# OminiX-ai/OminiX-MLX

Measured on AMD Instinct MI355X. Metric: decode_tokens_per_sec, higher is better.
Workload: dtype bf16

## Files before the change

### ominix-mlx_amd/csrc/attn_step.hip

```cpp
#include <algorithm>

#include "attn.hpp"
#include "act16.hpp"
#include "gemv_parts.hpp"
#include "granule.hpp"
#include "launch_timing.hpp"

namespace omx {

namespace {

constexpr int kBlock = 512;
constexpr int kWaves = 8;

template <int N>
__device__ __forceinline__ float swap_halves(float v) {
    if (N == 16) return dpp_f<0x128>(v);
    return dpp_f<0x1B>(dpp_f<kDppHalfMirror>(v));
}

template <bool F16 = false>
__device__ __forceinline__ void unpack8(const u32x4 r, float (&x)[8]) {
#pragma unroll
    for (int e = 0; e < 4; ++e) {
        x[2 * e] = Act16<F16>::lo(r[e]);
        x[2 * e + 1] = Act16<F16>::hi(r[e]);
    }
}

template <int D, int NB, bool F16 = false>
__device__ __forceinline__ void gather_head(const AttnStepArgs& a, const uint64_t* base, int n_active, unsigned tag, int lane,
                                            int dim, bf16_t* out, uint64_t* xg_head) {
    constexpr int STRIDE = D + 2;
    unsigned long long ml0 = 0, ml1 = 0, og[NB][16];
    bool ok_ml = false, ok_b[NB];
#pragma unroll
    for (int b = 0; b < NB; ++b) ok_b[b] = b * 16 >= n_active;
    const int sl = min(lane, n_active - 1);
    for (unsigned spins = 0;; ++spins) {
        if (!ok_ml) {
            ml0 = ld_granule(base + (size_t)sl * STRIDE + D);
            ml1 = ld_granule(base + (size_t)sl * STRIDE + D + 1);
        }
#pragma unroll
        for (int b = 0; b < NB; ++b) {
            if (ok_b[b]) continue;
#pragma unroll
            for (int j = 0; j < 16; ++j) og[b][j] = ld_granule(base + (size_t)min(b * 16 + j, n_active - 1) * STRIDE + dim);
        }
        bool all = true;
        if (!ok_ml) ok_ml = __all((unsigned)(ml0 >> 32) == tag && (unsigned)(ml1 >> 32) == tag);
        all = ok_ml;
#pragma unroll
        for (int b = 0; b < NB; ++b) {
            if (!ok_b[b]) {
                bool ok = true;
#pragma unroll
                for (int j = 0; j < 16; ++j) ok &= (unsigned)(og[b][j] >> 32) == tag;
                ok_b[b] = __all(ok);
            }
            all = all && ok_b[b];
        }
        if (all) break;
        if (spins >= kGranuleSpinLimit) {
            if (lane == 0) __hip_atomic_store(a.abort_flag, 1u, __ATOMIC_RELAXED, __HIP_MEMORY_SCOPE_AGENT);
            break;
        }
        __builtin_amdgcn_s_sleep(1);
    }
    const float m = lane < n_active ? __uint_as_float((unsigned)ml0) : -INFINITY;
    const float l = lane < n_active ? __uint_as_float((unsigned)ml1) : 0.f;
    const float M = wave_max(m);
    const float f = (m == -INFINITY) ? 0.f : __expf(m - M);
    const float L = wave_sum(f * l);
    float acc = 0.f;
#pragma unroll
    for (int b = 0; b < NB; ++b) {
        if (b * 16 >= n_active) break;
#pragma unroll
        for (int j = 0; j < 16; ++j)
            acc = fmaf(readlane_f(f, b * 16 + j), __uint_as_float((unsigned)og[b][j]), acc);
    }
    const bf16_t r = Act16<F16>::bits(acc / L);
    out[dim] = r;
    if (xg_head) {
        const float nb = dpp_f<kDppXor1>(bf16_to_f32(r));
        if (!(lane & 1)) st_granule_u32(xg_head + dim / 2, tag, (unsigned)r | ((unsigned)f32_to_bf16(nb) << 16));
    }
}

typedef __attribute__((ext_vector_type(2))) __bf16 bf16x2_t;
typedef __attribute__((ext_vector_type(2))) float f32x2;

typedef __attribute__((ext_vector_type(8))) __bf16 bf16x8_t;
__device__ __forceinline__ float dot8_bf16(const u32x4 a, const u32x4 b) {
    const bf16x8_t A = __builtin_bit_cast(bf16x8_t, a), B = __builtin_bit_cast(bf16x8_t, b);
    float d = 0.f;
    d = __builtin_amdgcn_fdot2_f32_bf16(__builtin_shufflevector(A, A, 0, 1), __builtin_shufflevector(B, B, 0, 1), d, false);
    d = __builtin_amdgcn_fdot2_f32_bf16(__builtin_shufflevector(A, A, 2, 3), __builtin_shufflevector(B, B, 2, 3), d, false);
    d = __builtin_amdgcn_fdot2_f32_bf16(__builtin_shufflevector(A, A, 4, 5), __builtin_shufflevector(B, B, 4, 5), d, false);
    d = __builtin_amdgcn_fdot2_f32_bf16(__builtin_shufflevector(A, A, 6, 7), __builtin_shufflevector(B, B, 6, 7), d, false);
    return d;
}

constexpr int kKU = 3;

template <bool F16>
__device__ __forceinline__ float dot8_16(const u32x4 a, const u32x4 b) {
    if constexpr (!F16) return dot8_bf16(a, b);
    float d = 0.f;
#pragma unroll
    for (int e = 0; e < 4; ++e) d = Act16<true>::dot2(a[e], b[e], d);
    return d;
}

constexpr int kORows = 4;

constexpr int kGuBlockPairs = 48, kGuHidden = 4096, kGuNV = kGuHidden / 512;
enum { kGuTicket = 0, kGuReduced = 1, kGuWords = 4 };

__device__ __forceinline__ int gateup_claim(int* sm_gu, int lane) {
    int t = 0;
    if (lane == 0) t = __hip_atomic_fetch_add(sm_gu + kGuTicket, 1, __ATOMIC_RELAXED, __HIP_MEMORY_SCOPE_WORKGROUP);
    return __builtin_amdgcn_readfirstlane(t);
}

__device__ __forceinline__ void gateup_issue(const AttnStepArgs& a, u32x4 (*w)[kGuNV], int pair, int lane) {
    const u32x4* g = reinterpret_cast<const u32x4*>(a.gu_gate + (size_t)pair * kGuHidden);
    const u32x4* u = reinterpret_cast<const u32x4*>(a.gu_up + (size_t)pair * kGuHidden);
#pragma unroll
    for (int j = 0; j < kGuNV; ++j) {
        w[0][j] = ld_nt(g + j * 64 + lane);
        w[1][j] = ld_nt(u + j * 64 + lane);
    }
    __builtin_amdgcn_sched_barrier(0);
}

template <int NVW>
__device__ __forceinline__ void oproj_await_vector(const AttnStepArgs& a, u32x4* sm_x, unsigned tag, int lane, int wave) {
    asm volatile("s_waitcnt vmcnt(0)" ::: "memory");
    if (wave == 0) {
        constexpr int SEGS = NVW * 8;
        const uint64_t* probe = a.xg + (size_t)min(lane, SEGS - 1) * 32 + 31;
        for (unsigned spins = 0; spins < kGranuleSpinLimit; ++spins) {
            const unsigned long long g = ld_granule(probe);
            if (__all((unsigned)(g >> 32) == tag)) break;
            __builtin_amdgcn_s_sleep(4);
        }
    }
    __syncthreads();
    constexpr int GP = (NVW + 1) / 2;
    static_assert((NVW * 256) % GP == 0, "a thread takes all of its granules or none");
    bool done = (int)threadIdx.x * GP >= NVW * 256;
    unsigned* sx = reinterpret_cast<unsigned*>(sm_x);
    for (unsigned spins = 0;; ++spins) {
        if (!done) {
            unsigned long long g[GP];
#pragma unroll
            for (int i = 0; i < GP; ++i) g[i] = ld_granule(a.xg + (size_t)threadIdx.x * GP + i);
            bool ok = true;
#pragma unroll
            for (int i = 0; i < GP; ++i) ok &= (unsigned)(g[i] >> 32) == tag;
            if (ok) {
#pragma unroll
                for (int i = 0; i < GP; ++i) sx[threadIdx.x * GP + i] = (unsigned)g[i];
                done = true;
            }
        }
        if (__syncthreads_and(done)) break;
        if (spins >= kGranuleSpinLimit) {
            if (threadIdx.x == 0) __hip_atomic_store(a.abort_flag, 1u, __ATOMIC_RELAXED, __HIP_MEMORY_SCOPE_AGENT);
            break;
        }
        __builtin_amdgcn_s_sleep(2);
    }
}

template <bool DN = false>
__device__ __forceinline__ void gateup_reduce(const AttnStepArgs& a, const u32x4 (*w)[kGuNV], const u32x4* xs, int pair, int lane,
                                              uint16_t* park = nullptr) {
    typedef Act16<false> A;
    float acc[2];
    rows_dot<false, 2, kGuNV>(w, xs, lane, acc);
    if constexpr (DN) {
        if (lane == 0) {
            const uint16_t v = epi_bits<EPI_SWIGLU, A>(acc[0], acc[1], (bf16_t)0, 0);
            a.gu_out[pair] = v;
            *park = v;
        }
    } else
    if (lane == 0) a.gu_out[pair] = epi_bits<EPI_SWIGLU, A>(acc[0], acc[1], (bf16_t)0, 0);
}

constexpr int kDnInter = 12288, kDnBlockRows = 16, kDnNV = kDnInter / 512 / 4, kDnUnits = kDnBlockRows / 2 * 4, kDnQRows = 3;
constexpr int kDnPartOff = kDnInter * 2, kDnParkOff = kDnPartOff + kDnBlockRows * 4 * 4, kDnLdsBytes = kDnParkOff + kGuBlockPairs * 2;
enum { kDnTicket = 4, kDnReduced = 5, kDnStored = 6, kDnWords = 8 };

__device__ __forceinline__ int down_claim(int* sm_gu, int lane) {
    int t = 0;
    if (lane == 0) t = __hip_atomic_fetch_add(sm_gu + kDnTicket, 1, __ATOMIC_RELAXED, __HIP_MEMORY_SCOPE_WORKGROUP);
    return __builtin_amdgcn_readfirstlane(t);
}

__device__ __forceinline__ void down_issue(const AttnStepArgs& a, u32x4 (*w)[kDnNV], int row_begin, int u, int lane) {
    const u32x4* p = reinterpret_cast<const u32x4*>(a.dn_w) + (size_t)(row_begin + 2 * (u >> 2)) * (kDnInter / 8) + (u & 3) * (kDnNV * 64) + lane;
#pragma unroll
    for (int r = 0; r < 2; ++r) {
#pragma unroll
        for (int j = 0; j < kDnNV; ++j) w[r][j] = ld_nt(p + (size_t)r * (kDnInter / 8) + j * 64);
    }
    __builtin_amdgcn_sched_barrier(0);
}

__device__ __forceinline__ void down_reduce(const u32x4 (*w)[kDnNV], const u32x4* xa, float* part, int u, int lane) {
    float acc[2];
    rows_dot<false, 2, kDnNV>(w, xa + (u & 3) * (kDnNV * 64), lane, acc);
    if (lane == 0) {
#pragma unroll
        for (int r = 0; r < 2; ++r) part[(2 * (u >> 2) + r) * 4 + (u & 3)] = acc[r];
    }
}

template <bool TRACE>
__device__ __forceinline__ void down_qkv_phase(const AttnStepArgs& a, unsigned char* sm_dn, u32x4* xs, float* red, int* sm_gu, unsigned res2,
                                               unsigned tag, int lane, int wave, unsigned long long* tr) {
    typedef Act16<false> A;
    u32x4* xa = reinterpret_cast<u32x4*>(sm_dn);
    float* part = reinterpret_cast<float*>(sm_dn + kDnPartOff);
    const int blk = (int)blockIdx.y * (int)gridDim.x + (int)blockIdx.x;
    const int row_begin = blk * kDnBlockRows;
    const int q_row0 = (blk * kWaves + __builtin_amdgcn_readfirstlane(wave)) * kDnQRows;
    constexpr int PV = kGuNV * 64 / 256;
    u32x4 nwv[PV];
#pragma unroll
    for (int i = 0; i < PV; ++i) nwv[i] = *(reinterpret_cast<const u32x4*>(a.nq_norm_w) + (threadIdx.x & 255) + i * 256);
    bf16_t ob[kDnQRows];
#pragma unroll
    for (int r = 0; r < kDnQRows; ++r) ob[r] = *(a.nq_bias ? a.nq_bias + min(q_row0 + r, a.nq.rows - 1) : a.nq_norm_w);
    u32x4 dA[2][kDnNV], dB[2][kDnNV];
    int tA = 0, tB = 0;
    u32x4 qw[kDnQRows][kGuNV];
    auto issue_qkv = [&](const int r0, const int r1) {
#pragma unroll
        for (int r = r0; r < r1; ++r) {
            const u32x4* p = reinterpret_cast<const u32x4*>(a.nq.row_ptr(min(q_row0 + r, a.nq.rows - 1), kGuHidden));
#pragma unroll
            for (int j = 0; j < kGuNV; ++j) qw[r][j] = ld_nt(p + j * 64 + lane);
        }
        __builtin_amdgcn_sched_barrier(0);
    };
    const bool sweeper = (wave & (kWaves / 2 - 1)) == 0;
    if (!sweeper) {
        tA = down_claim(sm_gu, lane);
        down_issue(a, dA, row_begin, tA, lane);
        tB = down_claim(sm_gu, lane);
        down_issue(a, dB, row_begin, tB, lane);
        issue_qkv(0, kDnQRows - 1);
    }
    lds_barrier();
    if (sweeper) {
        if (wave == 0 && lane < kGuBlockPairs / 2)
            st_granule_u32(a.ag + (size_t)blk * (kGuBlockPairs / 2) + lane, tag, reinterpret_cast<const unsigned*>(sm_dn + kDnParkOff)[lane]);
        sweep_granules<kDnInter / 2, 2>(a.ag, reinterpret_cast<unsigned*>(xa), __builtin_amdgcn_readfirstlane(wave) / (kWaves / 2), tag, lane, a.abort_flag);
        if (TRACE && threadIdx.x == 0) tr[11] = wall_clock64();
        tA = down_claim(sm_gu, lane);
        down_issue(a, dA, row_begin, tA, lane);
        tB = down_claim(sm_gu, lane);
        down_issue(a, dB, row_begin, tB, lane);
        issue_qkv(0, kDnQRows - 1);
    }
    lds_barrier();
    down_reduce(dA, xa, part, tA, lane);
    if (TRACE && threadIdx.x == 0) tr[12] = wall_clock64();
    int n_reduced = 1;
    int nA = down_claim(sm_gu, lane), nB;
    for (;;) {
        if (nA >= kDnUnits) {
            down_reduce(dB, xa, part, tB, lane);
            ++n_reduced;
            break;
        }
        tA = nA;
        down_issue(a, dA, row_begin, tA, lane);
        nB = down_claim(sm_gu, lane);
        down_reduce(dB, xa, part, tB, lane);
        if (nB >= kDnUnits) {
            down_reduce(dA, xa, part, tA, lane);
            n_reduced += 2;
            break;
        }
        tB = nB;
        down_issue(a, dB, row_begin, tB, lane);
        nA = down_claim(sm_gu, lane);
        down_reduce(dA, xa, part, tA, lane);
        n_reduced += 2;
    }
    if (TRACE && lane == 0) __hip_atomic_fetch_add(sm_gu + kDnReduced, n_reduced, __ATOMIC_RELAXED, __HIP_MEMORY_SCOPE_WORKGROUP);
    issue_qkv(kDnQRows - 1, kDnQRows);
    lds_barrier();
    if (wave == 0) {
        if (lane < kDnBlockRows / 2) {
            const uint32_t o2 = residual_pair<A, 4>(part + 2 * lane * 4, res2);
            reinterpret_cast<uint32_t*>(a.dn_out)[row_begin / 2 + lane] = o2;
            st_granule_u32(a.rg + row_begin / 2 + lane, tag, o2);
        }
        sweep_granules<kGuHidden / 2, 1>(a.rg, reinterpret_cast<unsigned*>(xs), 0, tag, lane, a.abort_flag);
        if (TRACE && lane == 0) tr[13] = wall_clock64();
    }
    lds_barrier();
    rmsnorm_in_lds<A, PV>(xs, red, nwv, kGuHidden, a.eps, threadIdx.x < 256);
    float acc[kDnQRows];
    rows_dot<false, kDnQRows, kGuNV>(qw, xs, lane, acc);
    if (lane == 0) {
        int stored = 0;
#pragma unroll
        for (int r = 0; r < kDnQRows; ++r)
            if (q_row0 + r < a.nq.rows) {
                a.nq_out[q_row0 + r] = A::bits(a.nq_bias ? acc[r] + A::val(ob[r]) : acc[r]);
                ++stored;
            }
        if (TRACE) __hip_atomic_fetch_add(sm_gu + kDnStored, stored, __ATOMIC_RELAXED, __HIP_MEMORY_SCOPE_WORKGROUP);
    }
    if constexpr (TRACE) {
        lds_barrier();
        if (threadIdx.x == 0) {
            tr[14] = wall_clock64();
            tr[15] = (unsigned long long)sm_gu[kDnReduced] | (unsigned long long)sm_gu[kDnStored] << 32;
        }
    }
}

template <bool TRACE, bool DN = false>
__device__ __forceinline__ void gateup_phase(const AttnStepArgs& a, u32x4* xs, float* red, int* sm_gu, const uint16_t* sm_pub, unsigned tag,
                                             int lane, int wave, int pub_row0, int pub_rows, unsigned long long* tr,
                                             unsigned char* sm_dn = nullptr) {
    typedef Act16<false> A;
    const int pair0 = ((int)blockIdx.y * (int)gridDim.x + (int)blockIdx.x) * kGuBlockPairs;
    uint16_t* park = DN ? reinterpret_cast<uint16_t*>(sm_dn + kDnParkOff) : nullptr;
    constexpr int PV = kGuNV * 64 / 256;
    u32x4 nwv[PV];
#pragma unroll
    for (int i = 0; i < PV; ++i) nwv[i] = *(reinterpret_cast<const u32x4*>(a.gu_norm_w) + (threadIdx.x & 255) + i * 256);
    u32x4 wA[2][kGuNV], wB[2][kGuNV];
    int tA = 0, tB;
    if (wave != 0) {
        tA = gateup_claim(sm_gu, lane);
        gateup_issue(a, wA, pair0 + tA, lane);
    }
    lds_barrier();
    if (wave == 0) {
        if (lane < pub_rows / 2) st_granule_u32(a.hg + pub_row0 / 2 + lane, tag, reinterpret_cast<const unsigned*>(sm_pub)[lane]);
        constexpr int GPL = kGuHidden / 2 / 64;
        for (unsigned spins = 0; spins < kGranuleSpinLimit; ++spins) {
            const unsigned long long g = ld_granule(a.hg + (size_t)lane * GPL + (GPL - 1));
            if (__all((unsigned)(g >> 32) == tag)) break;
            __builtin_amdgcn_s_sleep(4);
        }
        unsigned long long g[GPL];
#pragma unroll
        for (int i = 0; i < GPL; ++i) g[i] = ld_granule(a.hg + (size_t)i * 64 + lane);
        __builtin_amdgcn_sched_barrier(0);
        lds_barrier();
        tA = gateup_claim(sm_gu, lane);
        gateup_issue(a, wA, pair0 + tA, lane);
        unsigned bad = 0;
#pragma unroll
        for (int i = 0; i < GPL; ++i) bad |= (unsigned)(g[i] >> 32) ^ tag;
        asm volatile("; hidden row: tags read behind the first (gate, up) pair" : "+v"(bad));
        if (!__all(bad == 0)) {
            for (unsigned spins = 0;; ++spins) {
#pragma unroll
                for (int i = 0; i < GPL; ++i) g[i] = ld_granule(a.hg + (size_t)i * 64 + lane);
                bool ok = true;
#pragma unroll
                for (int i = 0; i < GPL; ++i) ok &= (unsigned)(g[i] >> 32) == tag;
                if (__all(ok)) break;
                if (spins >= kGranuleSpinLimit) {
                    if (lane == 0) __hip_atomic_store(a.abort_flag, 1u, __ATOMIC_RELAXED, __HIP_MEMORY_SCOPE_AGENT);
                    break;
                }
                __builtin_amdgcn_s_sleep(4);
            }
        }
        unsigned* sx = reinterpret_cast<unsigned*>(xs);
#pragma unroll
        for (int i = 0; i < GPL; ++i) sx[i * 64 + lane] = (unsigned)g[i];
        if (TRACE && lane == 0 && pub_rows > 0) tr[4] = wall_clock64();
        tB = gateup_claim(sm_gu, lane);
    } else {
        lds_barrier();
        tB = gateup_claim(sm_gu, lane);
        gateup_issue(a, wB, pair0 + tB, lane);
    }
    lds_barrier();
    unsigned res2 = 0;
    if constexpr (DN) res2 = reinterpret_cast<const unsigned*>(xs)[(pair0 / kGuBlockPairs) * (kDnBlockRows / 2) + (lane & (kDnBlockRows / 2 - 1))];
    rmsnorm_in_lds<A, PV>(xs, red, nwv, kGuHidden, a.eps, threadIdx.x < 256);
    if (wave == 0) {
        gateup_issue(a, wB, pair0 + tB, lane);
        gateup_reduce<DN>(a, wA, xs, pair0 + tA, lane, park + tA);
        if (TRACE && threadIdx.x == 0) tr[7] = wall_clock64();
        asm volatile("; first pair reduced: wave 0, its second pair just asked for" ::: "memory");
    } else {
        gateup_reduce<DN>(a, wA, xs, pair0 + tA, lane, park + tA);
        asm volatile("; first pair reduced: the second pair came in through the hop" ::: "memory");
    }
    int n_reduced = 1;
    int nA = gateup_claim(sm_gu, lane), nB;
    for (;;) {
        if (nA >= kGuBlockPairs) {
            gateup_reduce<DN>(a, wB, xs, pair0 + tB, lane, park + tB);
            ++n_reduced;
            break;
        }
        tA = nA;
        gateup_issue(a, wA, pair0 + tA, lane);
        nB = gateup_claim(sm_gu, lane);
        gateup_reduce<DN>(a, wB, xs, pair0 + tB, lane, park + tB);
        if (nB >= kGuBlockPairs) {
            gateup_reduce<DN>(a, wA, xs, pair0 + tA, lane, park + tA);
            n_reduced += 2;
            break;
        }
        tB = nB;
        gateup_issue(a, wB, pair0 + tB, lane);
        nA = gateup_claim(sm_gu, lane);
        gateup_reduce<DN>(a, wA, xs, pair0 + tA, lane, park + tA);
        n_reduced += 2;
    }
    if constexpr (TRACE) {
        if (lane == 0) {
            __hip_atomic_fetch_add(sm_gu + kGuReduced, n_reduced, __ATOMIC_RELAXED, __HIP_MEMORY_SCOPE_WORKGROUP);
            if (wave == 0) tr[8] = wall_clock64();
            if (wave == kWaves - 1) tr[9] = wall_clock64();
        }
        lds_barrier();
        if (threadIdx.x == 0) tr[10] = (unsigned long long)sm_gu[kGuReduced];
    }
    if constexpr (DN) down_qkv_phase<TRACE>(a, sm_dn, xs, red, sm_gu, res2, tag, lane, wave, tr);
}

template <int NVW, int R, bool GU = false>
__device__ __forceinline__ void oproj_phase(const AttnStepArgs& a, u32x4* sm_x, unsigned tag, int lane, int wave, int o_row0,
                                            unsigned long long* tr, uint16_t* sm_pub = nullptr, int pub_row0 = 0) {
    u32x4 ow[R][NVW];
#pragma unroll
    for (int r = 0; r < R; ++r) {
        const int row = min(o_row0 + r, a.o_rows - 1);
        const u32x4* p = reinterpret_cast<const u32x4*>(a.o_w + (size_t)row * (NVW * 512));
#pragma unroll
        for (int j = 0; j < NVW; ++j) ow[r][j] = __builtin_nontemporal_load(p + j * 64 + lane);
    }
    bf16_t o_res[R];
#pragma unroll
    for (int r = 0; r < R; ++r) o_res[r] = a.o_resid[min(o_row0 + r, a.o_rows - 1)];
    __builtin_amdgcn_sched_barrier(0);
    oproj_await_vector<NVW>(a, sm_x, tag, lane, wave);
    if (tr && threadIdx.x == 0) tr[5] = wall_clock64();
    float acc[R];
    rows_dot<false, R, NVW>(ow, sm_x, lane, acc);
    if (lane == 0) {
#pragma unroll
        for (int r = 0; r < R; ++r)
            if (o_row0 + r < a.o_rows) {
                if (a.o_out_f32) a.o_out_f32[o_row0 + r] = acc[r];
                else {
                    const bf16_t hb = f32_to_bf16(bf16_to_f32(o_res[r]) + round_bf16(acc[r]));
                    a.o_out[o_row0 + r] = hb;
                    if (GU) sm_pub[o_row0 + r - pub_row0] = hb;
                }
            }
    }
    if (tr && threadIdx.x == 0) tr[6] = wall_clock64();
}


template <int NVW, int R>
__device__ __forceinline__ void oproj_phase_q4(const AttnStepArgs& a, u32x4* sm_x, float* sm_xsum, unsigned tag, int lane, int wave,
                                               int o_row0, unsigned long long* tr) {
    static_assert(NVW % 4 == 0, "K must be a multiple of 2048");
    constexpr int ST = NVW / 4;
    u32x4 ow[R][ST];
    uint32_t sbv[R][ST];
    const int words_per_row = NVW * 64, groups_per_row = NVW * 512 / a.o_group;
#pragma unroll
    for (int r = 0; r < R; ++r) {
        const int row = min(o_row0 + r, a.o_rows - 1);
        const uint32_t* p = a.o_wq + (size_t)row * words_per_row;
        const uint32_t* psb = a.o_sb + (size_t)row * groups_per_row;
#pragma unroll
        for (int st = 0; st < ST; ++st) {
            const int chunk = st * 64 + lane;
            ow[r][st] = __builtin_nontemporal_load(reinterpret_cast<const u32x4*>(p + (size_t)chunk * 4));
            sbv[r][st] = psb[chunk * 32 / a.o_group];
        }
    }
    bf16_t o_res[R];
#pragma unroll
    for (int r = 0; r < R; ++r) o_res[r] = a.o_resid[min(o_row0 + r, a.o_rows - 1)];
    __builtin_amdgcn_sched_barrier(0);
    oproj_await_vector<NVW>(a, sm_x, tag, lane, wave);
    if ((int)threadIdx.x < NVW * 64) {
        const u32x4 o = sm_x[threadIdx.x];
        u32x4 t;
        t[0] = __builtin_amdgcn_perm(o[1], o[0], 0x05040100u); t[1] = __builtin_amdgcn_perm(o[3], o[2], 0x05040100u);
        t[2] = __builtin_amdgcn_perm(o[1], o[0], 0x07060302u); t[3] = __builtin_amdgcn_perm(o[3], o[2], 0x07060302u);
        sm_x[threadIdx.x] = t;
        float sv = 0.f;
#pragma unroll
        for (int q = 0; q < 4; ++q) sv += bf16lo(o[q]) + bf16hi(o[q]);
        sv += dpp_f<kDppXor1>(sv);
        sv += dpp_f<kDppXor2>(sv);
        if ((threadIdx.x & 3) == 0) sm_xsum[threadIdx.x >> 2] = sv;
    }
    __syncthreads();
    if (tr && threadIdx.x == 0) tr[5] = wall_clock64();
    float acc[R];
#pragma unroll
    for (int r = 0; r < R; ++r) acc[r] = 0.f;
#pragma unroll
    for (int st = 0; st < ST; ++st) {
        const int chunk = st * 64 + lane;
        uint32_t xp[16];
#pragma unroll
        for (int j = 0; j < 4; ++j) {
            const u32x4 xv = sm_x[chunk * 4 + j];
#pragma unroll
            for (int q = 0; q < 4; ++q) xp[j * 4 + q] = xv[q];
        }
        const float xsm = sm_xsum[chunk];
#pragma unroll
        for (int r = 0; r < R; ++r) {
            float d = 0.f;
            const float scl = bf16lo(sbv[r][st]);
            float bia = bf16hi(sbv[r][st]);
#pragma unroll
            for (int wi = 0; wi < 4; ++wi) {
                const uint32_t wdw = ow[r][st][wi];
                const uint32_t lo = wdw & 0x0F0F0F0Fu, hi = (wdw >> 4) & 0x0F0F0F0Fu;
                const uint32_t c43 = 0x43434343u;
                const uint32_t q0 = __builtin_amdgcn_perm(c43, lo, 0x04010400u), q1 = __builtin_amdgcn_perm(c43, lo, 0x04030402u);
                const uint32_t q2 = __builtin_amdgcn_perm(c43, hi, 0x04010400u), q3 = __builtin_amdgcn_perm(c43, hi, 0x04030402u);
                d = __builtin_amdgcn_fdot2_f32_bf16(__builtin_bit_cast(bf16x2_t, xp[wi * 4 + 0]), __builtin_bit_cast(bf16x2_t, q0), d, false);
                d = __builtin_amdgcn_fdot2_f32_bf16(__builtin_bit_cast(bf16x2_t, xp[wi * 4 + 1]), __builtin_bit_cast(bf16x2_t, q1), d, false);
                d = __builtin_amdgcn_fdot2_f32_bf16(__builtin_bit_cast(bf16x2_t, xp[wi * 4 + 2]), __builtin_bit_cast(bf16x2_t, q2), d, false);
                d = __builtin_amdgcn_fdot2_f32_bf16(__builtin_bit_cast(bf16x2_t, xp[wi * 4 + 3]), __builtin_bit_cast(bf16x2_t, q3), d, false);
            }
            bia = fmaf(-128.0f, scl, bia);
            acc[r] = fmaf(scl, d, acc[r]);
            acc[r] = fmaf(bia, xsm, acc[r]);
        }
    }
#pragma unroll
    for (int r = 0; r < R; ++r) acc[r] = wave_sum(acc[r]);
    if (lane == 0) {
#pragma unroll
        for (int r = 0; r < R; ++r)
            if (o_row0 + r < a.o_rows) a.o_out[o_row0 + r] = f32_to_bf16(bf16_to_f32(o_res[r]) + round_bf16(acc[r]));
    }
    if (tr && threadIdx.x == 0) tr[6] = wall_clock64();
}


template <int D, int GT, bool TRACE, int NVW, bool F16 = false, bool GU = false, bool DN = false>
__global__ __launch_bounds__(kBlock, 1) void attn_step_kernel(const AttnStepArgs a) {
    static_assert(!DN || GU, "down + the next q/k/v follow gate/up only");
    static_assert(!F16 || NVW == 0, "the O projection rides in the launch for bfloat16 models only");
    static_assert(!GU || (NVW == kGuNV && D == 128), "gate/up follows the bf16 O projection of hidden 4096 only");
    typedef Act16<F16> A16;
    constexpr int LPR = D / 8;
    constexpr int TPW = 64 / LPR;
    constexpr bool QO = NVW >= 100;
    constexpr int NV = QO ? NVW - 100 : NVW;
    constexpr bool OPROJ = NV > 0;
    extern __shared__ __attribute__((aligned(16))) unsigned char smem[];
    float* sm_o = reinterpret_cast<float*>(smem);
    float* sm_m = sm_o + kWaves * TPW * GT * D;
    float* sm_l = sm_m + kWaves * GT;
    u32x4* sm_q = reinterpret_cast<u32x4*>(sm_l + kWaves * GT);
    u32x4* sm_x = sm_q + (GT + 1) * LPR;
    float* sm_xsum = reinterpret_cast<float*>(sm_x + NV * 64);
    int* sm_gu = reinterpret_cast<int*>(sm_x + NV * 64);

    const int lane = threadIdx.x & 63;
    const int wave = threadIdx.x >> 6;
    const int c = lane % LPR;
    const int sg = lane / LPR;
    const int kvh = blockIdx.x, split = blockIdx.y;
    const int G = a.H / a.Hkv;
    unsigned long long* tr = TRACE ? a.trace + ((size_t)split * a.Hkv + kvh) * kAttnTraceWords : nullptr;
    if (TRACE && threadIdx.x == 0) tr[0] = wall_clock64();
    if constexpr (GU) {
        if (threadIdx.x < (DN ? kDnWords : kGuWords)) sm_gu[threadIdx.x] = 0;
    }

    bf16_t* Kb = a.k + (size_t)kvh * a.kv_head_stride;
    bf16_t* Vb = a.v + (size_t)kvh * a.kv_head_stride;
    const int t_begin = split * a.chunk;
    const int n_units = a.chunk / TPW;

    const bf16_t* kraw = a.qkv + (size_t)a.H * D + (size_t)kvh * D;
    const bool does_q = wave < GT, does_k = wave == GT % kWaves;
    const bf16_t* my_raw = does_q ? a.qkv + (size_t)(kvh * G + min(wave, G - 1)) * D : kraw;
    const u32x4 raw0 = *reinterpret_cast<const u32x4*>(my_raw + c * 8);
    const u32x4 raw1 = *reinterpret_cast<const u32x4*>(kraw + c * 8);
    const u32x4 vnew = *reinterpret_cast<const u32x4*>(kraw + (size_t)a.Hkv * D + c * 8);
    const int i0 = (c % (LPR / 2)) * 8;
    const f32x4* cp = reinterpret_cast<const f32x4*>(a.rope_cur + i0);
    const f32x4* sp = reinterpret_cast<const f32x4*>(a.rope_cur + D / 2 + i0);
    const f32x4 c0 = cp[0], c1 = cp[1], s0 = sp[0], s1 = sp[1];
    u32x4 wq_raw = {0, 0, 0, 0}, wk_raw = {0, 0, 0, 0};
    if (a.q_norm_w) {
        wq_raw = *reinterpret_cast<const u32x4*>(a.q_norm_w + c * 8);
        wk_raw = *reinterpret_cast<const u32x4*>(a.k_norm_w + c * 8);
    }
    u32x4 kr[kKU], vr[kKU];
    auto issue_kv = [&](int u0) {
#pragma unroll
        for (int u = 0; u < kKU; ++u) {
            const int tc = min(t_begin + (u0 + u * kWaves) * TPW + sg, a.cap - 1);
            kr[u] = *reinterpret_cast<const u32x4*>(Kb + (size_t)tc * D + c * 8);
            vr[u] = *reinterpret_cast<const u32x4*>(Vb + (size_t)tc * D + c * 8);
        }
    };
    issue_kv(wave);
    const int pos = *a.pos_ptr;
    const unsigned tag = *a.seq_ptr * a.tag_mul + a.tag_add;

    {
        float cs[8], sn[8];
#pragma unroll
        for (int e = 0; e < 4; ++e) {
            cs[e] = c0[e]; cs[4 + e] = c1[e];
            sn[e] = s0[e]; sn[4 + e] = s1[e];
        }
        const bool first_half = c < LPR / 2;
        auto norm_rope = [&](const u32x4 raw, const u32x4 w_raw) -> u32x4 {
            float x[8], w[8];
            unpack8<F16>(raw, x);
            unpack8<F16>(w_raw, w);
            float ss = 0.f;
#pragma unroll
            for (int e = 0; e < 8; ++e) ss = fmaf(x[e], x[e], ss);
            ss = group_sum<LPR>(ss);
            const float rstd = a.q_norm_w ? 1.0f / sqrtf(ss / (float)D + a.eps) : 1.0f;
            float y[8];
#pragma unroll
            for (int e = 0; e < 8; ++e) {
                const float xn = a.q_norm_w ? A16::rnd(x[e] * rstd * w[e]) : x[e];
                const float other = swap_halves<LPR>(xn);
                y[e] = first_half ? xn * cs[e] - other * sn[e] : other * sn[e] + xn * cs[e];
            }
            u32x4 out;
#pragma unroll
            for (int e = 0; e < 4; ++e) out[e] = A16::pack(y[2 * e], y[2 * e + 1]);
            return out;
        };
        if (does_q && sg == 0) sm_q[wave * LPR + c] = norm_rope(raw0, wq_raw);
        if (does_k && sg == 0) sm_q[GT * LPR + c] = norm_rope(does_q ? raw1 : raw0, wk_raw);
    }
    asm volatile("s_waitcnt lgkmcnt(0)\n\ts_barrier" ::: "memory");
    u32x4 q[GT];
#pragma unroll
    for (int g = 0; g < GT; ++g) q[g] = sm_q[g * LPR + c];
    const u32x4 knew = sm_q[GT * LPR + c];

    const int Tk = pos + 1;
    const int n_active = (Tk + a.chunk - 1) / a.chunk;
    const int t_end = min(Tk, t_begin + a.chunk);
    const bool active = split < n_active;
    if (TRACE && threadIdx.x == 0) tr[1] = wall_clock64();

    float m[GT], l[GT];
    f32x2 o[GT][4];
#pragma unroll
    for (int g = 0; g < GT; ++g) {
        m[g] = -INFINITY;
        l[g] = 0.f;
#pragma unroll
        for (int e = 0; e < 4; ++e) o[g][e] = f32x2{0.f, 0.f};
    }
    auto round = [&](const int u0) {
        float s[kKU][GT];
        f32x2 vf[kKU][4];
#pragma unroll
        for (int u = 0; u < kKU; ++u) {
            const int unit = u0 + u * kWaves;
            const int tok = t_begin + unit * TPW + sg;
            const bool live = unit < n_units && tok < t_end;
            u32x4 kp = kr[u], vp = vr[u];
            if (tok == pos && unit < n_units) {
                kp = knew;
                vp = vnew;
                *reinterpret_cast<u32x4*>(Kb + (size_t)pos * D + c * 8) = kp;
                *reinterpret_cast<u32x4*>(Vb + (size_t)pos * D + c * 8) = vp;
            }
#pragma unroll
            for (int e = 0; e < 4; ++e)
                vf[u][e] = live ? f32x2{A16::lo(vp[e]), A16::hi(vp[e])} : f32x2{0.f, 0.f};
#pragma unroll
            for (int g = 0; g < GT; ++g) {
                const float d = group_sum<LPR>(dot8_16<F16>(q[g], kp)) * a.scale;
                s[u][g] = live ? d : -INFINITY;
            }
        }
        if (u0 + kWaves * kKU < n_units && t_begin + (u0 + kWaves * kKU) * TPW < t_end) issue_kv(u0 + kWaves * kKU);
#pragma unroll
        for (int g = 0; g < GT; ++g) {
            float mx = s[0][g];
#pragma unroll
            for (int u = 1; u < kKU; ++u) mx = fmaxf(mx, s[u][g]);
            float wmx = readlane_f(mx, 0);
#pragma unroll
            for (int r = 1; r < TPW; ++r) wmx = fmaxf(wmx, readlane_f(mx, r * LPR));
            const float mn = fmaxf(m[g], wmx);
            const float alpha = (mn == -INFINITY) ? 1.f : __expf(m[g] - mn);
            m[g] = mn;
            l[g] *= alpha;
            const f32x2 al = {alpha, alpha};
#pragma unroll
            for (int e = 0; e < 4; ++e) o[g][e] *= al;
#pragma unroll
            for (int u = 0; u < kKU; ++u) {
                const float p = (mn == -INFINITY) ? 0.f : __expf(s[u][g] - mn);
                l[g] += p;
                const f32x2 pp = {p, p};
#pragma unroll
                for (int e = 0; e < 4; ++e) o[g][e] = __builtin_elementwise_fma(pp, vf[u][e], o[g][e]);
            }
        }
    };
    if (wave < n_units && t_begin + wave * TPW < t_end) round(wave);
    for (int u0 = wave + kWaves * kKU; u0 < n_units && t_begin + u0 * TPW < t_end; u0 += kWaves * kKU) round(u0);
    if (TRACE && threadIdx.x == 0) tr[2] = wall_clock64();

    if (active) {
#pragma unroll
        for (int g = 0; g < GT; ++g) {
            float* dst = sm_o + (((size_t)(wave * TPW + sg) * GT + g) * D + c * 8);
            *reinterpret_cast<f32x4*>(dst) = f32x4{o[g][0][0], o[g][0][1], o[g][1][0], o[g][1][1]};
            *reinterpret_cast<f32x4*>(dst + 4) = f32x4{o[g][2][0], o[g][2][1], o[g][3][0], o[g][3][1]};
            float lw = readlane_f(l[g], 0);
#pragma unroll
            for (int r = 1; r < TPW; ++r) lw += readlane_f(l[g], r * LPR);
            if (lane == 0) {
                sm_m[wave * GT + g] = m[g];
                sm_l[wave * GT + g] = lw;
            }
        }
        __syncthreads();
        if (TRACE && !GU && threadIdx.x == 0) tr[7] = wall_clock64();
        for (int idx = threadIdx.x; idx < G * D; idx += kBlock) {
            const int g = idx / D, d = idx % D;
            float M = sm_m[g];
#pragma unroll
            for (int w = 1; w < kWaves; ++w) M = fmaxf(M, sm_m[w * GT + g]);
            float L = 0.f, O = 0.f;
#pragma unroll
            for (int w = 0; w < kWaves; ++w) {
                const float mw = sm_m[w * GT + g];
                const float f = (mw == -INFINITY) ? 0.f : __expf(mw - M);
                float ow = 0.f;
#pragma unroll
                for (int r = 0; r < TPW; ++r) ow += sm_o[((size_t)(w * TPW + r) * GT + g) * D + d];
                L = fmaf(f, sm_l[w * GT + g], L);
                O = fmaf(f, ow, O);
            }
            uint64_t* gr = a.ws + ((size_t)(kvh * G + g) * a.nsplit + split) * (D + 2);
            st_granule(gr + d, tag, O);
            if (d == 0) {
                st_granule(gr + D, tag, M);
                st_granule(gr + D + 1, tag, L);
            }
        }
    }
    if (TRACE && threadIdx.x == 0) tr[3] = wall_clock64();

    if (OPROJ && split >= G) {
        const int g = ((split - G) * (int)gridDim.x + kvh) * kWaves + wave;
        const bool hi = g < a.o_nhi;
        const int rows = hi ? a.o_rpw : a.o_rpw - 1;
        const int o_row0 = hi ? g * a.o_rpw : a.o_nhi * a.o_rpw + (g - a.o_nhi) * (a.o_rpw - 1);
        unsigned long long* otr = TRACE ? tr : nullptr;
        if constexpr (GU) {
            auto row0_of = [&](int w) { return w < a.o_nhi ? w * a.o_rpw : a.o_nhi * a.o_rpw + (w - a.o_nhi) * (a.o_rpw - 1); };
            const int pub_row0 = row0_of(g - wave), pub_rows = row0_of(g - wave + kWaves) - pub_row0;
            uint16_t* sm_pub = reinterpret_cast<uint16_t*>(sm_l);
            if (rows == 2) oproj_phase<NV, 2, true>(a, sm_x, tag, lane, wave, o_row0, otr, sm_pub, pub_row0);
            else oproj_phase<NV, 3, true>(a, sm_x, tag, lane, wave, o_row0, otr, sm_pub, pub_row0);
            gateup_phase<TRACE, DN>(a, sm_x, sm_m, sm_gu, sm_pub, tag, lane, wave, pub_row0, pub_rows, otr, smem);
            return;
        } else
        if constexpr (QO) {
            if (rows <= 1) oproj_phase_q4<NV, 1>(a, sm_x, sm_xsum, tag, lane, wave, o_row0, otr);
            else if (rows == 2) oproj_phase_q4<NV, 2>(a, sm_x, sm_xsum, tag, lane, wave, o_row0, otr);
            else if (rows == 3) oproj_phase_q4<NV, 3>(a, sm_x, sm_xsum, tag, lane, wave, o_row0, otr);
            else oproj_phase_q4<NV, 4>(a, sm_x, sm_xsum, tag, lane, wave, o_row0, otr);
        } else {
            if (rows <= 1) oproj_phase<(NV > 0 ? NV : 1), 1>(a, sm_x, tag, lane, wave, o_row0, otr);
            else if (rows == 2) oproj_phase<(NV > 0 ? NV : 1), 2>(a, sm_x, tag, lane, wave, o_row0, otr);
            else if (rows == 3) oproj_phase<(NV > 0 ? NV : 1), 3>(a, sm_x, tag, lane, wave, o_row0, otr);
            else oproj_phase<(NV > 0 ? NV : 1), 4>(a, sm_x, tag, lane, wave, o_row0, otr);
        }
        return;
    }

    if (split < G && wave < D / 64) {
        const int head = kvh * G + split;
        const uint64_t* base = a.ws + (size_t)head * a.nsplit * (D + 2);
        bf16_t* out = a.out + (size_t)head * D;
        const int dim = wave * 64 + lane;
        const int nb = (a.nsplit + 15) / 16;
        uint64_t* xg_head = OPROJ ? a.xg + (size_t)head * (D / 2) : nullptr;
        if (nb <= 1) gather_head<D, 1, F16>(a, base, n_active, tag, lane, dim, out, xg_head);
        else if (nb == 2) gather_head<D, 2, F16>(a, base, n_active, tag, lane, dim, out, xg_head);
        else gather_head<D, 3, F16>(a, base, n_active, tag, lane, dim, out, xg_head);
        if (TRACE && threadIdx.x == 0) tr[4] = wall_clock64();
    }
    if constexpr (GU) {
        lds_barrier();
        gateup_phase<TRACE, DN>(a, sm_x, sm_m, sm_gu, nullptr, tag, lane, wave, 0, 0, TRACE ? tr : nullptr, smem);
    }
}

}

int attn_step_block_tokens(int D) { return 64 / (D / 8); }

constexpr int kMaxSplits = 48;
void attn_step_plan(int tk_max, int Hkv, int G, int D, int* chunk, int* nsplit) {
    const int unit = attn_step_block_tokens(D);
    int target = std::max(1, std::min(kMaxSplits, 256 / std::max(Hkv, 1)));
    if (const char* v = getenv("OMX_ATTN_STEP_SPLITS")) target = std::max(1, std::min(kMaxSplits, atoi(v)));
    int ch = unit * ((tk_max + unit * target - 1) / (unit * target));
    if (ch < unit) ch = unit;
    int ns = (tk_max + ch - 1) / ch;
    if (ns < G) ns = G;
    *chunk = ch;
    *nsplit = ns;
}

size_t attn_step_ws_granules(int H, int D) { return (size_t)H * kMaxSplits * (D + 2); }

static int oproj_rows_per_wave(int H, int Hkv, int nsplit, int o_rows) {
    const int waves = (Hkv * nsplit - H) * kWaves;
    return waves > 0 ? (o_rows + waves - 1) / waves : 1 << 20;
}
bool attn_step_oproj_ok(int H, int Hkv, int D, int nsplit, int o_rows) {
    const int K = H * D, nvw = K / 512;
    return K % 512 == 0 && (nvw == 1 || nvw == 2 || nvw == 4 || nvw == 7 || nvw == 8) && oproj_rows_per_wave(H, Hkv, nsplit, o_rows) <= kORows;
}

bool attn_step_oproj_q4_ok(int H, int Hkv, int D, int nsplit, int o_rows, int group) {
    const int K = H * D;
    return (K == 2048 || K == 4096) && (group == 32 || group == 64 || group == 128) && attn_step_oproj_ok(H, Hkv, D, nsplit, o_rows);
}

bool attn_step_gateup_ok(int H, int Hkv, int D, int nsplit, int o_rows, int gu_rows) {
    const int blocks = Hkv * nsplit, waves = (blocks - H) * kWaves;
    if (D != 128 || H * D != kGuHidden || o_rows != kGuHidden || H / std::max(Hkv, 1) != 4 || blocks != 256) return false;
    if (gu_rows != blocks * kGuBlockPairs || !attn_step_oproj_ok(H, Hkv, D, nsplit, o_rows)) return false;
    return oproj_rows_per_wave(H, Hkv, nsplit, o_rows) == 3 && (o_rows - waves * 2) % kWaves == 0;
}

bool attn_step_down_ok(int o_rows, int gu_rows, int nq_rows) {
    const int waves = 256 * kWaves;
    return o_rows == 256 * kDnBlockRows && gu_rows == kDnInter && nq_rows > (kDnQRows - 1) * waves && nq_rows <= kDnQRows * waves;
}

template <int D, int GT, bool TRACE, int NVW, bool F16 = false, bool GU = false, bool DN = false>
static int launch_instance(dim3 grid, size_t shmem, hipStream_t s, const AttnStepArgs& a) {
    if (shmem > 48 * 1024)
        OMX_HIP_CHECK(hipFuncSetAttribute((const void*)attn_step_kernel<D, GT, TRACE, NVW, F16, GU, DN>, hipFuncAttributeMaxDynamicSharedMemorySize, (int)shmem));
    OMX_LAUNCH_TIMED((attn_step_kernel<D, GT, TRACE, NVW, F16, GU, DN>), grid, dim3(kBlock), shmem, s, a);
    OMX_LAUNCH_CHECK();
    return 0;
}

int launch_attn_step(const AttnStepArgs& a_in, int D, hipStream_t s) {
    AttnStepArgs a = a_in;
    const int G = a.H / a.Hkv;
    OMX_REQUIRE(a.H % a.Hkv == 0 && G >= 1 && G <= 8, "decode attention: %d query heads over %d KV heads unsupported (group of at most 8)", a.H, a.Hkv);
    OMX_REQUIRE(a.nsplit >= G && a.nsplit <= kMaxSplits && a.chunk > 0 && a.chunk % attn_step_block_tokens(D) == 0 && a.Hkv * a.nsplit <= 256,
                "decode attention: bad split plan (chunk %d, %d splits, group %d, %d kv heads)", a.chunk, a.nsplit, G, a.Hkv);
    OMX_REQUIRE(a.ws && a.rope_cur && a.pos_ptr && a.seq_ptr && a.abort_flag && a.tag_mul > a.tag_add - 1u && a.tag_add >= 1u,
                "decode attention: missing step state");
    int nvw = 0;
    const bool qo = a.o_wq != nullptr;
    if (qo)
        OMX_REQUIRE(!a.o_w && a.o_sb && a.o_out && !a.o_out_f32 && attn_step_oproj_q4_ok(a.H, a.Hkv, D, a.nsplit, a.o_rows, a.o_group),
                    "decode attention + packed O projection: shape does not qualify (H*D = %d, group %d)", a.H * D, a.o_group);
    if (a.o_w || qo) {
        OMX_REQUIRE(a.o_resid && (a.o_out || a.o_out_f32) && a.xg && attn_step_oproj_ok(a.H, a.Hkv, D, a.nsplit, a.o_rows),
                    "decode attention + O projection: shape does not qualify (H*D = %d, %d rows, %d blocks)", a.H * D, a.o_rows, a.Hkv * a.nsplit);
        nvw = a.H * D / 512;
        a.o_rpw = oproj_rows_per_wave(a.H, a.Hkv, a.nsplit, a.o_rows);
        const int waves = (a.Hkv * a.nsplit - a.H) * kWaves;
        a.o_nhi = a.o_rpw > 1 ? a.o_rows - waves * (a.o_rpw - 1) : waves;
    }
    if (a.gu_gate)
        OMX_REQUIRE(a.o_w && a.o_out && !a.o_out_f32 && !a.f16 && a.gu_up && a.gu_norm_w && a.gu_out && a.hg &&
                        attn_step_gateup_ok(a.H, a.Hkv, D, a.nsplit, a.o_rows, a.gu_rows),
                    "decode attention + gate/up: shape does not qualify (%d blocks, %d O rows, %d pairs)", a.Hkv * a.nsplit, a.o_rows, a.gu_rows);
    if (a.dn_w)
        OMX_REQUIRE(a.gu_gate && a.dn_out && a.ag && a.rg && a.nq.w0 && a.nq.w1 && a.nq.w2 && a.nq_norm_w && a.nq_out &&
                        a.nq.n0 > 0 && a.nq.n1 > 0 && a.nq.rows > a.nq.n0 + a.nq.n1 && attn_step_down_ok(a.o_rows, a.gu_rows, a.nq.rows),
                    "decode attention + down + q/k/v: shape does not qualify (%d rows, %d pairs, %d q/k/v rows)", a.o_rows, a.gu_rows, a.nq.rows);
    const dim3 grid(a.Hkv, a.nsplit);
    const int gt = G <= 1 ? 1 : G <= 2 ? 2 : G <= 4 ? 4 : 8;
#define OMX_ATTN_STEP_CASE(DD, GG)                                                                                       \
    if (D == DD && gt == GG) {                                                                                           \
        const size_t shmem = ((size_t)kWaves * (64 / (DD / 8)) * GG * DD + 2 * kWaves * GG) * sizeof(float) +            \
                             (size_t)(GG + 1) * (DD / 8) * 16 + (size_t)nvw * 64 * 16 + (qo ? (size_t)nvw * 64 : 0) +    \
                             (a.dn_w ? kDnWords * sizeof(int) : a.gu_gate ? kGuWords * sizeof(int) : 0);                 \
        if (a.gu_gate) {                            \
            if constexpr (DD == 128 && GG == 4) {                                                                        \
                static_assert(kDnLdsBytes <= kWaves * 4 * 4 * 128 * 4, "the down phase lives in the split-merge area");  \
                if (a.dn_w && a.trace) return launch_instance<128, 4, true, kGuNV, false, true, true>(grid, shmem, s, a); \
                if (a.dn_w) return launch_instance<128, 4, false, kGuNV, false, true, true>(grid, shmem, s, a);          \
                if (a.trace) return launch_instance<128, 4, true, kGuNV, false, true>(grid, shmem, s, a);                \
                return launch_instance<128, 4, false, kGuNV, false, true>(grid, shmem, s, a);                            \
            }                                                                                                            \
            return set_error("decode attention + gate/up: no instantiation for head_dim %d, group %d", DD, GG);         \
        }                                                                                                                \
        if (a.trace && !qo) {                           \
            if (nvw == 0) return launch_instance<DD, GG, true, 0>(grid, shmem, s, a);                                    \
            if (nvw == 8) return launch_instance<DD, GG, true, 8>(grid, shmem, s, a);                                    \
            return set_error("decode attention: no traced instantiation for H*D = %d", a.H * DD);                       \
        }                                                                                                                \
        if (qo) {                                                                                                        \
            if (nvw == 4) return launch_instance<DD, GG, false, 104>(grid, shmem, s, a);                                 \
            return launch_instance<DD, GG, false, 108>(grid, shmem, s, a);                                               \
        }                                                                                                                \
        if (a.f16) {    \
            if constexpr (DD == 128) {                                                                                   \
                if (nvw == 0) return launch_instance<DD, GG, false, 0, true>(grid, shmem, s, a);                         \
            }                                                                                                            \
            return set_error("decode attention: float16 models take head_dim 128 without the O projection in the launch"); \
        }                                                                                                                \
        if (nvw == 0) return launch_instance<DD, GG, false, 0>(grid, shmem, s, a);                                       \
        if (nvw == 1) return launch_instance<DD, GG, false, 1>(grid, shmem, s, a);                                       \
        if (nvw == 2) return launch_instance<DD, GG, false, 2>(grid, shmem, s, a);                                       \
        if (nvw == 4) return launch_instance<DD, GG, false, 4>(grid, shmem, s, a);                                       \
        if (nvw == 7) return launch_instance<DD, GG, false, 7>(grid, shmem, s, a);                                       \
        return launch_instance<DD, GG, false, 8>(grid, shmem, s, a);                                                     \
    }
    OMX_ATTN_STEP_CASE(128, 1) OMX_ATTN_STEP_CASE(128, 2) OMX_ATTN_STEP_CASE(128, 4) OMX_ATTN_STEP_CASE(128, 8)
    OMX_ATTN_STEP_CASE(64, 1) OMX_ATTN_STEP_CASE(64, 2) OMX_ATTN_STEP_CASE(64, 4) OMX_ATTN_STEP_CASE(64, 8)
#undef OMX_ATTN_STEP_CASE
    return set_error("decode attention: head_dim %d unsupported (64 or 128)", D);
}

}
```

Measured before the change: 353.5.

## Overlap granule sweep with first down-projection weight loads in sweeper waves

Sweeper waves now publish the block's granule before the barrier. They spin only on the last granule per lane, issue the granule loads, then claim and issue the first down-projection unit before checking the tags, so the activation fetch latency overlaps the weight loads. A fallback respins on any stale tag and sets the abort flag after the limit. Non-sweeper waves split their QKV weight prefetch around an extra barrier to match the new barrier count, which adds barriers and more complex synchronisation.

```diff
diff --git a/ominix-mlx_amd/csrc/attn_step.hip b/ominix-mlx_amd/csrc/attn_step.hip
--- a/ominix-mlx_amd/csrc/attn_step.hip
+++ b/ominix-mlx_amd/csrc/attn_step.hip
@@ -250,24 +250,60 @@
         __builtin_amdgcn_sched_barrier(0);
     };
     const bool sweeper = (wave & (kWaves / 2 - 1)) == 0;
-    if (!sweeper) {
+    lds_barrier();
+    if (wave == 0 && lane < kGuBlockPairs / 2)
+        st_granule_u32(a.ag + (size_t)blk * (kGuBlockPairs / 2) + lane, tag, reinterpret_cast<const unsigned*>(sm_dn + kDnParkOff)[lane]);
+    lds_barrier();
+    if (sweeper) {
+        constexpr int HALF = kDnInter / 2 / 2, GPL = HALF / 64;
+        const int half = __builtin_amdgcn_readfirstlane(wave) / (kWaves / 2);
+        const uint64_t* gr = a.ag + (size_t)half * HALF;
+        for (unsigned spins = 0; spins < kGranuleSpinLimit; ++spins) {
+            const unsigned long long g = ld_granule(gr + (size_t)lane * GPL + (GPL - 1));
+            if (__all((unsigned)(g >> 32) == tag)) break;
+            __builtin_amdgcn_s_sleep(4);
+        }
+        unsigned long long g[GPL];
+#pragma unroll
+        for (int i = 0; i < GPL; ++i) g[i] = ld_granule(gr + (size_t)i * 64 + lane);
+        __builtin_amdgcn_sched_barrier(0);
+        lds_barrier();
+        tA = down_claim(sm_gu, lane);
+        down_issue(a, dA, row_begin, tA, lane);
+        unsigned bad = 0;
+#pragma unroll
+        for (int i = 0; i < GPL; ++i) bad |= (unsigned)(g[i] >> 32) ^ tag;
+        asm volatile("; activation vector: tags read behind the first down unit" : "+v"(bad));
+        if (!__all(bad == 0)) {
+            for (unsigned spins = 0;; ++spins) {
+#pragma unroll
+                for (int i = 0; i < GPL; ++i) g[i] = ld_granule(gr + (size_t)i * 64 + lane);
+                bool ok = true;
+#pragma unroll
+                for (int i = 0; i < GPL; ++i) ok &= (unsigned)(g[i] >> 32) == tag;
+                if (__all(ok)) break;
+                if (spins >= kGranuleSpinLimit) {
+                    if (lane == 0) __hip_atomic_store(a.abort_flag, 1u, __ATOMIC_RELAXED, __HIP_MEMORY_SCOPE_AGENT);
+                    break;
+                }
+                __builtin_amdgcn_s_sleep(4);
+            }
+        }
+        unsigned* sx = reinterpret_cast<unsigned*>(xa) + half * HALF;
+#pragma unroll
+        for (int i = 0; i < GPL; ++i) sx[i * 64 + lane] = (unsigned)g[i];
+        if (TRACE && threadIdx.x == 0) tr[11] = wall_clock64();
+        tB = down_claim(sm_gu, lane);
+        down_issue(a, dB, row_begin, tB, lane);
+        issue_qkv(0, kDnQRows - 1);
+    } else {
         tA = down_claim(sm_gu, lane);
         down_issue(a, dA, row_begin, tA, lane);
         tB = down_claim(sm_gu, lane);
         down_issue(a, dB, row_begin, tB, lane);
-        issue_qkv(0, kDnQRows - 1);
-    }
-    lds_barrier();
-    if (sweeper) {
-        if (wave == 0 && lane < kGuBlockPairs / 2)
-            st_granule_u32(a.ag + (size_t)blk * (kGuBlockPairs / 2) + lane, tag, reinterpret_cast<const unsigned*>(sm_dn + kDnParkOff)[lane]);
-        sweep_granules<kDnInter / 2, 2>(a.ag, reinterpret_cast<unsigned*>(xa), __builtin_amdgcn_readfirstlane(wave) / (kWaves / 2), tag, lane, a.abort_flag);
-        if (TRACE && threadIdx.x == 0) tr[11] = wall_clock64();
-        tA = down_claim(sm_gu, lane);
-        down_issue(a, dA, row_begin, tA, lane);
-        tB = down_claim(sm_gu, lane);
-        down_issue(a, dB, row_begin, tB, lane);
-        issue_qkv(0, kDnQRows - 1);
+        issue_qkv(0, 1);
+        lds_barrier();
+        issue_qkv(1, kDnQRows - 1);
     }
     lds_barrier();
     down_reduce(dA, xa, part, tA, lane);
```

New measurement: 358.5 (median of 6 runs). +1.4%, better.
